# jimonld2000/AudioDenoiser

Measured on AMD Instinct MI355X. Metric: spectrogram frames/sec (forward), 513x256 fp32, higher is better.
Workload: dtype f32; 1 GPU; BASELINE configs[1]: batch=64 synthetic 513x256 fp32 spectrograms on one MI355X, full U-Net forward + per-clip perceptual loss; batch_per_gpu=64, global_batch=64, freq_bins=513, frames=256, parallelism=clips sharded over 1 rank(s), weights replicated, no data-path collective, lib_digest=616623384a0f

## Files before the change

### audiodenoiser_amd/csrc/adn_internal.h

```cpp
#pragma once
#include <hip/hip_runtime.h>
#include <atomic>
#include <cstddef>
#include <cstdint>
#include <type_traits>

namespace adn {

template <typename T> constexpr int ACT_BLOCK = 32 / (int)sizeof(T);
template <typename T>
__host__ __device__ __forceinline__ long act_off(int C, long HW, long pix, int c)
{
    constexpr int B = ACT_BLOCK<T>;
    (void)C;
    return ((long)(c / B) * HW + pix) * B + (c % B);
}

#ifdef __HIPCC__
typedef float f32x2 __attribute__((ext_vector_type(2)));
typedef float f32x4 __attribute__((ext_vector_type(4)));
typedef float f32x16 __attribute__((ext_vector_type(16)));
typedef _Float16 f16x2 __attribute__((ext_vector_type(2)));
typedef _Float16 f16x4 __attribute__((ext_vector_type(4)));
typedef _Float16 f16x8 __attribute__((ext_vector_type(8)));
// ... 207 lines not shown
}
inline int device_cus()
{
    static std::atomic<int> cus{0};
    int c = cus.load(std::memory_order_relaxed);
    if (c == 0) {
        int dev = 0;
        if (hipGetDevice(&dev) != hipSuccess || hipDeviceGetAttribute(&c, hipDeviceAttributeMultiprocessorCount, dev) != hipSuccess || c < 8)
            return 0;
        c &= ~7;
        cus.store(c, std::memory_order_relaxed);
    }
    return c;
}

hipError_t launch_conv_mfma(ConvKind kind, const ConvArgs &a, bool f16, hipStream_t st);
hipError_t launch_conv_reduce(ConvKind kind, const ConvArgs &a, bool f16, hipStream_t st);
hipError_t launch_convt_reduce(const float *partial, const float *bias, float *out, int ksplit, int N, int Ho, int Wo, int Cout,
                               hipStream_t st);
constexpr int WINO_BN = 32;
hipError_t launch_wino_conv(ConvKind kind, const ConvArgs &a, hipStream_t st);
long wino_tiles(ConvArgs &a);
bool wino4_applicable(ConvKind kind, const ConvArgs &a, bool force);
long wino4_workgroups(const ConvArgs &a);
hipError_t launch_wino4_conv(ConvKind kind, const ConvArgs &a, hipStream_t st);

struct Wino3sGeom {
    int tilesY, tilesX;
    long rows;
    size_t v_bytes, m_bytes;
    long gemm_grid;
};
enum SplitTile { SPLIT_BN128 = 0, SPLIT_BN256 = 1, SPLIT_BN256W8 = 2 };
inline int split_tile_bn(SplitTile t) { return t == SPLIT_BN128 ? 128 : 256; }
bool wino3s_applicable(ConvKind kind, const ConvArgs &a);
Wino3sGeom wino3s_geom(const ConvArgs &a);
hipError_t launch_wino3s_conv(ConvKind kind, const ConvArgs &a, float *V, float *M, SplitTile tile, hipStream_t st);
hipError_t launch_wino_gemm(const float *V, const void *U, float *M, long rows, int Cin, int Cout, SplitTile tile, hipStream_t st);

bool conv16_applicable(ConvKind kind, const ConvArgs &a);
hipError_t launch_conv16(ConvKind kind, const ConvArgs &a, bool resident, hipStream_t st);

bool convt16_applicable(const ConvArgs &a);
hipError_t launch_convt16(const ConvArgs &a, hipStream_t st);

hipError_t launch_conv_first(const float *x, const float *w9x64, const float *bias, void *out, bool f16,
                             int N, int H, int W, int Cin, hipStream_t st);
hipError_t launch_dot_finish(const float *planes, int nplanes, float bias, float *y, long npix, hipStream_t st);
hipError_t launch_conv_out(const void *in, bool f16, const float *w64, float bias, float *out, long npix, long HW,
                           long out_stride, hipStream_t st);
hipError_t launch_nhwc_to_nchw(const void *in, bool f16, float *out, int N, int H, int W, int C, hipStream_t st);

hipError_t launch_stft_mag(const float *audio, int n_clips, long L, int n_fft, int hop, int center, long n_frames,
// ... 204 lines not shown
```

### audiodenoiser_amd/csrc/conv_kernels.hip

```cpp
#include "adn_internal.h"

#include <cstdlib>

namespace adn {

namespace {

constexpr int TW = 16;
constexpr int CONVT_KG = 2, CONVT_WPE = 4;

template <typename T> struct Elem;
template <> struct Elem<float> { static constexpr int EPV = 4; };
template <> struct Elem<_Float16> { static constexpr int EPV = 8; };

template <int TH, int BN, int WM, int WN>
__device__ __forceinline__ void conv_epilogue_raw(const ConvArgs &p, f32x16 (&acc)[TH * TW / 32 / WM][BN / 32 / WN], int lane, int wave,
                                                  int ct, int n, int ty, int tx)
{
    constexpr int MB = TH * TW / 32 / WM, NB = BN / 32 / WN;
    const int wm = wave / WN, wn = wave % WN;
    const int hh = lane >> 5, l31 = lane & 31;
    float *ob = static_cast<float *>(p.out) + (size_t)n * p.H * p.W * p.Cout;
#pragma unroll
    for (int j = 0; j < NB; ++j) {
// ... 369 lines not shown
                    const T *b0 = stage + ((2 * ly) * TW + 2 * lx) * RS + part * EPP;
                    piece_t m = *reinterpret_cast<const piece_t *>(b0);
                    const piece_t m1 = *reinterpret_cast<const piece_t *>(b0 + RS);
                    const piece_t m2 = *reinterpret_cast<const piece_t *>(b0 + TW * RS);
                    const piece_t m3 = *reinterpret_cast<const piece_t *>(b0 + TW * RS + RS);
                    m = __builtin_elementwise_maximum(__builtin_elementwise_maximum(m, m1), __builtin_elementwise_maximum(m2, m3));
                    *reinterpret_cast<piece_t *>(poolp + (size_t)n * Hp * Wp * p.Cout +
                                                 act_off<T>(p.Cout, (long)Hp * Wp, (long)py * Wp + px, ct * BN + part * EPP)) = m;
                }
            }
        }
    }
    }
}

template <typename T, int TH, int BN, int WM, int WN, int TAPS, int KG, int SPLIT = 0>
struct DmaCfg {
    static constexpr int NT = 64 * WM * WN;
    static constexpr int HALO = (TAPS == 9) ? 1 : 0;
    static constexpr int PH = TH + 2 * HALO, PW = TW + 2 * HALO;
    static constexpr int KQ = 2 * KG;
    static constexpr int PSLOT = (KG == 1) ? KQ : KQ + 1;
    static constexpr int RSLOT = PW * PSLOT + ((KG == 1) ? 1 : 0);
    static constexpr int A_USED = PH * RSLOT;
    static constexpr int A_SLOTS = (A_USED + 63) / 64 * 64;
    static constexpr int B_SLOTS = SPLIT ? TAPS * 3 * 2 * BN : TAPS * KG * 2 * BN;
    static constexpr int SLOTS = A_SLOTS + B_SLOTS;
    static constexpr int NPIECE = (SLOTS + NT - 1) / NT;
    static constexpr int A_ROUNDS = (A_SLOTS + NT - 1) / NT;
    static constexpr size_t LDS_BYTES = (size_t)2 * SLOTS * 16;
    static_assert(B_SLOTS % 64 == 0, "weight slab must be a whole number of wave copies");
};

template <typename T, int TH, int BN, int WM, int WN, int TAPS, int KG, int EPI, int WPE, int SPLIT = 0, int KSPLIT = 0>
__global__ __launch_bounds__(64 * WM * WN, WPE) void conv_dma(const ConvArgs p)
{
    using C = DmaCfg<T, TH, BN, WM, WN, TAPS, KG, SPLIT>;
    static_assert(!KSPLIT || EPI == CONVT2X2 || (sizeof(T) == 2 && EPI == CONV3X3_RELU), "K split: transposed convolutions, fp16 3x3 layers");
    static_assert(!SPLIT || (sizeof(T) == 4 && KG == 2 && TAPS == 1), "SPLIT: fp32 storage, one 16-channel chunk (two fp32 k-groups), 1 tap");
    constexpr bool GEMM = EPI == WINO_GEMM;
    static_assert(!GEMM || (SPLIT && !KSPLIT && TW == 16), "Winograd GEMM stage: split-bf16 form");
    constexpr int NT = C::NT, EPV = Elem<T>::EPV, HALO = C::HALO, PW = C::PW;
    static_assert(2 * EPV == ACT_BLOCK<T>, "one k-group = one channel block of the activation layout");
    constexpr int PSLOT = C::PSLOT, RSLOT = C::RSLOT, A_SLOTS = C::A_SLOTS, SLOTS = C::SLOTS, NPIECE = C::NPIECE;
    constexpr int A_ROUNDS = C::A_ROUNDS;
    constexpr int B_DW = C::B_SLOTS * 4;
    constexpr int MB = TH * TW / 32 / WM, NB = BN / 32 / WN;
    static_assert(WM * WN == 4 || WM * WN == 8, "4 or 8 waves per workgroup");
    static_assert(MB >= 1 && NB >= 1, "tile too small");

    extern __shared__ __attribute__((aligned(16))) float smem[];

// ... 36 lines not shown
    unsigned cstr = (unsigned)((size_t)KG * src_hw(p.s0) * ACT_BLOCK<T> * sizeof(T));
    unsigned wsoff = 0;
    const int c0 = KSPLIT ? ksp * nloc : 0;
    bool in2 = false;
    if constexpr (KSPLIT) {
        wsoff = (unsigned)c0 * (unsigned)(B_DW * 4);
        if (c0 > p.nchunk0) {
            in2 = true;
            cstr = (unsigned)((size_t)KG * p.s1.H * p.s1.W * ACT_BLOCK<T> * sizeof(T));
            hptr = src_base(p.s1) + (size_t)(c0 - p.nchunk0) * cstr;
        } else {
            hptr += (size_t)c0 * cstr;
        }
    }
    const unsigned loff = lane * 16;
    unsigned hcur[A_ROUNDS];
    auto dma_piece = [&](int k, int buf, bool want_a, bool want_b) {
        const int sb = k * NT + wave * 64;
        if (sb >= SLOTS) return;
        float *dst = smem + (size_t)buf * SLOTS * 4 + sb * 4;
        if (k < A_ROUNDS && sb < A_SLOTS) {
            if (want_a) dma16_buf(dma_rsrc(hptr, cstr), hcur[k < A_ROUNDS ? k : 0], 0u, dst);
        } else if (want_b) {
            dma16_buf(wrs, loff, wsoff + (unsigned)(sb - A_SLOTS) * 16u, dst);
        }
    };
#pragma unroll
    for (int k = 0; k < NPIECE; ++k) dma_piece(k, 0, false, true);

    auto plan = [&](const ConvSrc &src) {
#pragma unroll
// ... 25 lines not shown
    float bias_r[NB];
#pragma unroll
    for (int j = 0; j < NB; ++j) bias_r[j] = GEMM ? 0.f : p.bias[ct * BN + (wn * NB + j) * 32 + l31];

    f32x16 acc[MB][NB];
#pragma unroll
    for (int i = 0; i < MB; ++i)
#pragma unroll
        for (int j = 0; j < NB; ++j)
#pragma unroll
            for (int r = 0; r < 16; ++r) acc[i][j][r] = 0.f;

    const int a_lane = ((wm * MB * 2 + ((lane >> 4) & 1)) * RSLOT + (lane & 15) * PSLOT) * 4 + hh * 4;
    const int b_lane = A_SLOTS * 4 + hh * BN * 4 + (wn * NB * 32 + l31) * 4;

    dma_chunk(c0, 0, false);
    asm volatile("s_waitcnt vmcnt(0)" ::: "memory");
    __syncthreads();
    for (int c = c0; c < c0 + nloc; ++c) {
        if (c + 1 < c0 + nloc) dma_chunk(c + 1, (c + 1 - c0) & 1);
        const float *img = smem + (size_t)((c - c0) & 1) * SLOTS * 4;
        if constexpr (SPLIT) {
            bf16x8 ah[MB], am[MB], al[MB];
#pragma unroll
            for (int i = 0; i < MB; ++i) {
                const float *ap = img + a_lane + (i * 2 * RSLOT) * 4 + hh * 4;
                split3_bf16(*reinterpret_cast<const f32x4 *>(ap), *reinterpret_cast<const f32x4 *>(ap + 4), ah[i], am[i], al[i]);
            }
#pragma unroll
            for (int j = 0; j < NB; ++j) {
// ... 31 lines not shown
#pragma unroll
                            for (int j = 0; j < NB; ++j)
                                acc[i][j] = __builtin_amdgcn_mfma_f32_32x32x2f32(a[i][kk], b[j][kk], acc[i][j], 0, 0, 0);
                } else {
#pragma unroll
                    for (int i = 0; i < MB; ++i)
#pragma unroll
                        for (int j = 0; j < NB; ++j)
                            acc[i][j] = __builtin_amdgcn_mfma_f32_32x32x16_f16(__builtin_bit_cast(f16x8, a[i]),
                                                                               __builtin_bit_cast(f16x8, b[j]), acc[i][j], 0, 0, 0);
                }
            }
        }
        asm volatile("s_waitcnt vmcnt(0)" ::: "memory");
        __syncthreads();
    }
    if constexpr (KSPLIT && EPI != CONVT2X2) {
        conv_epilogue_raw<TH, BN, WM, WN>(p, acc, lane, wave, ct, n + ksp * p.N, ty, tx);
    } else if constexpr (sizeof(T) == 2 || EPI == CONVT2X2 || GEMM) {
        constexpr size_t tile = (size_t)TH * TW * (BN + 16 / sizeof(T)) * sizeof(T);
        constexpr int HALVES = tile <= C::LDS_BYTES ? 1 : 2;
        static_assert(tile / HALVES <= C::LDS_BYTES, "staging tile (or half of it) must fit the two images");
        conv_epilogue_staged<T, TH, BN, WM, WN, EPI, HALVES>(p, acc, bias_r, smem, tid, lane, wave, ct, KSPLIT ? n + ksp * p.N : n, ty, tx);
    } else {
        conv_epilogue<T, TH, BN, WM, WN, EPI>(p, acc, bias_r, lane, wave, ct, n, ty, tx);
    }
}

constexpr int FIRST_ROWS = 8;

// ... 124 lines not shown
    }
}

template <typename T, int TH, int BN, int WM, int WN, int TAPS, int KG, int EPI>
hipError_t launch_cfg(const ConvArgs &a, hipStream_t st)
{
    constexpr int HALO = (TAPS == 9) ? 1 : 0;
    constexpr int PH = TH + 2 * HALO, PW = TW + 2 * HALO;
    constexpr size_t lds = (size_t)(PH * PW * (8 * KG + 4) + TAPS * KG * 2 * BN * 4) * sizeof(float);
    const long nwg = conv_workgroups(a);
    if (nwg <= 0 || nwg > 0x7fffffffL) return hipErrorInvalidValue;
    hipLaunchKernelGGL((conv_mfma<T, TH, BN, WM, WN, TAPS, KG, EPI>), dim3((unsigned)nwg), dim3(64 * WM * WN), lds, st, a);
    return hipGetLastError();
}

template <typename T, int TH, int BN, int WM, int WN, int TAPS, int KG, int EPI, int WPE, int SPLIT = 0, int KSPLIT = 0>
hipError_t launch_dma_cfg(const ConvArgs &a, hipStream_t st)
{
    using C = DmaCfg<T, TH, BN, WM, WN, TAPS, KG, SPLIT>;
    const long nwg = conv_workgroups(a);
    const int ks = KSPLIT ? a.ksplit : 1;
    if (nwg <= 0 || ks < 1 || nwg * ks > 0x7fffffffL || a.nchunk % ks) return hipErrorInvalidValue;
    ConvArgs a2 = a;
    a2.nwg_base = (int)nwg;
    a2.fdGc = a2.fdNcg = a2.fdTx = a2.fdTy = FastDiv{0u, 0u};
    const long maxd = a.nct > a.tilesX ? (a.nct > a.tilesY ? a.nct : a.tilesY) : (a.tilesX > a.tilesY ? a.tilesX : a.tilesY);
    if ((unsigned long long)nwg * (unsigned long long)maxd < 0x100000000ull) {
        a2.fdGc = make_fastdiv((unsigned)a.nct);
        a2.fdTx = make_fastdiv((unsigned)a.tilesX);
        a2.fdTy = make_fastdiv((unsigned)a.tilesY);
    }
    constexpr auto kern = conv_dma<T, TH, BN, WM, WN, TAPS, KG, EPI, WPE, SPLIT, KSPLIT>;
    if (C::LDS_BYTES > 64 * 1024) {
        const hipError_t e = lds_opt_in<kern>(C::LDS_BYTES);
        if (e != hipSuccess) return e;
    }
    hipLaunchKernelGGL(kern, dim3((unsigned)(nwg * ks)), dim3(C::NT), C::LDS_BYTES, st, a2);
    return hipGetLastError();
}

__global__ __launch_bounds__(256) void convt_reduce_kernel(const f32x4 *__restrict__ partial, const float *__restrict__ bias,
                                                           f32x4 *__restrict__ out, int ksplit, long n4, long hw, int cblocks)
{
    const long i = (long)blockIdx.x * 256 + threadIdx.x;
    if (i >= n4) return;
    const int c = (int)((i / (2 * hw)) % cblocks) * 8 + (int)(i & 1) * 4;
    f32x4 t[ADN_MAX_KSPLIT];
// ... 52 lines not shown
        for (int a = 0; a < 2; ++a)
#pragma unroll
            for (int b = 0; b < 2; ++b) {
                const int gy = 2 * by + a, gx = 2 * bx + b;
                if (gy >= H || gx >= W) continue;
                const f32x4 v = finish(gy, gx);
                mx.x = max_nan(mx.x, v.x); mx.y = max_nan(mx.y, v.y); mx.z = max_nan(mx.z, v.z); mx.w = max_nan(mx.w, v.w);
            }
        if (by < H / 2 && bx < W / 2)
            *reinterpret_cast<Tx4 *>(pool + (size_t)n * (H / 2) * (W / 2) * Cout +
                                     act_off<T>(Cout, (long)(H / 2) * (W / 2), (long)by * (W / 2) + bx, c4)) = as_t(mx);
    }
}

template <typename T>
hipError_t launch_conv_mfma_t(ConvKind kind, const ConvArgs &a, hipStream_t st)
{
    if constexpr (sizeof(T) == 2) {
        if (a.ksplit > 1) {
            if (kind != CONV3X3_RELU) return hipErrorInvalidValue;
            return launch_dma_cfg<T, 32, 64, 8, 1, 9, 1, CONV3X3_RELU, 4, 0, 1>(a, st);
        }
        if (kind == CONVT2X2) return launch_dma_cfg<T, 8, 128, 2, 2, 1, CONVT_KG, CONVT2X2, CONVT_WPE>(a, st);
        if (kind == CONV3X3_RELU_DOT) {
            if (a.nct != 1 || !a.dotw || !a.dot_out) return hipErrorInvalidValue;
            return launch_dma_cfg<T, 32, 64, 8, 1, 9, 1, CONV3X3_RELU_DOT, 4>(a, st);
        }
        if (kind == CONV3X3_RELU_POOL) return launch_dma_cfg<T, 32, 64, 8, 1, 9, 1, CONV3X3_RELU_POOL, 4>(a, st);
        return launch_dma_cfg<T, 32, 64, 8, 1, 9, 1, CONV3X3_RELU, 4>(a, st);
    } else {
        if (kind == CONV3X3_RELU_DOT) return hipErrorInvalidValue;
        if (kind == CONVT2X2) {
            if (a.split > 1 && a.ksplit > 1) return hipErrorInvalidValue;
            if (a.split && a.ksplit > 1) return launch_dma_cfg<T, 8, 128, 2, 2, 1, CONVT_KG, CONVT2X2, 3, 1, 1>(a, st);
            if (a.ksplit > 1) return hipErrorInvalidValue;
            if (a.split == 1 + SPLIT_BN256) return launch_dma_cfg<T, 8, 256, 2, 2, 1, CONVT_KG, CONVT2X2, 2, 1>(a, st);
            if (a.split == 1 + SPLIT_BN256W8) return launch_dma_cfg<T, 8, 256, 2, 4, 1, CONVT_KG, CONVT2X2, 2, 1>(a, st);
            if (a.split) return launch_dma_cfg<T, 8, 128, 2, 2, 1, CONVT_KG, CONVT2X2, 3, 1>(a, st);
            return launch_dma_cfg<T, 8, 128, 2, 2, 1, CONVT_KG, CONVT2X2, CONVT_WPE>(a, st);
        }
        if (a.Cout == 64) {
            if (kind == CONV3X3_RELU_POOL) return launch_cfg<T, 16, 64, 4, 1, 9, 1, CONV3X3_RELU_POOL>(a, st);
            return launch_cfg<T, 16, 64, 4, 1, 9, 1, CONV3X3_RELU>(a, st);
        }
        if (kind == CONV3X3_RELU_POOL) return launch_cfg<T, 8, 128, 2, 2, 9, 1, CONV3X3_RELU_POOL>(a, st);
        return launch_cfg<T, 8, 128, 2, 2, 9, 1, CONV3X3_RELU>(a, st);
    }
}
// ... 6 lines not shown
    if (kind == CONVT2X2) return ConvGeom{8, 128, CONVT_KG * cpg};
    if (f16) return ConvGeom{32, 64, cpg};
    if (Cout == 64) return ConvGeom{16, 64, cpg};
    return ConvGeom{8, 128, cpg};
}

long conv_mfma_tiles(ConvKind kind, bool f16, ConvArgs &a)
{
    const ConvGeom g = conv_geom(kind, a.Cout, f16);
    a.tilesY = (a.H + g.TH - 1) / g.TH;
    a.tilesX = (a.W + TW - 1) / TW;
    a.nct = (kind == CONVT2X2 ? 4 * a.Cout : a.Cout) / g.BN;
    return conv_workgroups(a);
}

hipError_t launch_conv_mfma(ConvKind kind, const ConvArgs &a, bool f16, hipStream_t st)
{
    return f16 ? launch_conv_mfma_t<_Float16>(kind, a, st) : launch_conv_mfma_t<float>(kind, a, st);
}

hipError_t launch_wino_gemm(const float *V, const void *U, float *M, long rows, int Cin, int Cout, SplitTile tile, hipStream_t st)
{
    const int BN = split_tile_bn(tile);
    if (!V || !U || !M || rows < 1 || rows >= (1L << 25) || Cin < 16 || (Cin & 15) || Cout < BN || Cout % BN) return hipErrorInvalidValue;
    ConvArgs a{};
    a.N = 36;
    a.W = TW;
    a.H = (int)((rows + TW - 1) / TW);
    a.rows = rows;
    a.s0 = ConvSrc{V, a.H, a.W, Cin, 0, 0};
    a.s1 = ConvSrc{V, 0, 0, 0, 0, 0};
    a.nchunk0 = a.nchunk = Cin / 16;
    a.wpk = U;
    a.out = M;
    a.Cout = Cout;
    a.ksplit = 1;
    a.split = 1;
    a.tilesY = (a.H + 7) / 8;
    a.tilesX = 1;
    a.nct = Cout / BN;
    if (tile == SPLIT_BN256) return launch_dma_cfg<float, 8, 256, 2, 2, 1, CONVT_KG, WINO_GEMM, 2, 1>(a, st);
    if (tile == SPLIT_BN256W8) return launch_dma_cfg<float, 8, 256, 2, 4, 1, CONVT_KG, WINO_GEMM, 2, 1>(a, st);
    return launch_dma_cfg<float, 8, 128, 2, 2, 1, CONVT_KG, WINO_GEMM, 3, 1>(a, st);
}

template <typename T>
static hipError_t launch_conv_reduce_t(bool pl, const ConvArgs &a, unsigned blocks, hipStream_t st)
{
    if (pl)
        hipLaunchKernelGGL((conv_reduce_kernel<T, true>), dim3(blocks), dim3(256), 0, st, a.partial, a.bias, static_cast<T *>(a.out),
                           static_cast<T *>(a.pool), a.ksplit, a.N, a.H, a.W, a.Cout);
    else
        hipLaunchKernelGGL((conv_reduce_kernel<T, false>), dim3(blocks), dim3(256), 0, st, a.partial, a.bias, static_cast<T *>(a.out),
                           static_cast<T *>(nullptr), a.ksplit, a.N, a.H, a.W, a.Cout);
    return hipGetLastError();
// ... 89 lines not shown
```

### audiodenoiser_amd/csrc/unet.hip

```cpp
#include "adn_host.h"

#include <algorithm>
#include <cmath>
#include <cstdlib>
#include <cstring>
#include <memory>
#include <vector>

using adn::aligned_to;
using adn::DeviceGuard;
using adn::fail;
using adn::fail_hip;

namespace {

constexpr float BN_EPS = 1e-5f;
constexpr int CH[5] = {64, 128, 256, 512, 1024};

enum LayerKind { CONV3, CONVT };
struct LayerDesc {
    LayerKind kind;
    int level;
    int C0, C1;
    int Cout;
// ... 49 lines not shown
    std::vector<hipEvent_t> events;
    int timing_max = 0, timing_count = 0;
    bool f16 = false;
    bool use_wino = true;
    bool use_wino4 = true, force_wino4 = false;
    bool allow_split = false;
    bool convt_split = true;
    int f16_conv = 1;
    int f16_convt = 1;
    bool f16_fuse_first = true;
    bool batch_invariant = false;
    long auto_grid = 192, auto_grid64 = 512;
    int wino_gemm = 1;
    long gemm_grid = 1536;
    int split_bn = -1;
    long convt_wide_grid = 2048;
};

namespace {

void bn_fold(const float *b, const float *gamma, const float *beta, const float *mean, const float *var, int C,
             std::vector<float> &scale, std::vector<float> &bias)
{
    scale.resize(C);
    bias.resize(C);
    for (int c = 0; c < C; ++c) {
        const float s = gamma[c] / std::sqrt(var[c] + BN_EPS);
        scale[c] = s;
        bias[c] = (b[c] - mean[c]) * s + beta[c];
    }
// ... 289 lines not shown
adn::ConvArgs convt_args(const adn_unet *h, const Plan &p, int i, const void *in, void *out)
{
    const LayerDesc &d = NET.v[i];
    const int H = p.H[d.level], W = p.W[d.level];
    adn::ConvArgs a = geom_args(d, h->f16, false, p.N, H, W);
    a.s0 = adn::ConvSrc{in, H, W, d.C0, 0, 0};
    a.s1 = adn::ConvSrc{in, 0, 0, 0, 0, 0};
    a.wpk = h->dev + h->lw[i].w_off;
    a.bias = h->dev + h->lw[i].b_off;
    a.out = out;
    a.split = h->convt_split ? 1 : 0;
    return a;
}


enum Conv3Kernel {
    DIRECT,
    CONV16,
    WINO2,
    WINO4,
    WINO3S
};
struct WinoScratch {
    const void *U = nullptr;
    adn::SplitTile tile = adn::SPLIT_BN128;
    float *V = nullptr, *M = nullptr;
    size_t v_bytes = 0, m_bytes = 0;
};
struct Conv3Choice {
    Conv3Kernel kernel;
    int ksplit;
    bool fuse_first;
    bool fuse_out;
};

Conv3Choice choose_conv3(const adn_unet *h, adn::ConvKind kind, const adn::ConvArgs &a, bool first = false, bool tail = false,
                         const WinoScratch &sc = WinoScratch())
{
    Conv3Choice c{DIRECT, 1, false, false};
    if (h->f16) {
// ... 52 lines not shown
                c.kernel = WINO4;
                c.ksplit = ks4;
            }
        }
    }
    return done();
}

hipError_t launch_conv3_kernels(const adn_unet *h, adn::ConvKind kind, const Conv3Choice &c, adn::ConvArgs a, float *partial, hipStream_t st,
                                const WinoScratch &sc)
{
    if (c.fuse_out) kind = adn::CONV3X3_RELU_DOT;
    switch (c.kernel) {
    case WINO3S:
        a.wpk = sc.U;
        return adn::launch_wino3s_conv(kind, a, sc.V, sc.M, sc.tile, st);
    case CONV16:
        a.wpk = a.wpk4;
        a.nchunk0 = a.s0.C / 32;
        a.nchunk = (a.s0.C + a.s1.C) / 32;
        if (c.fuse_first) a.nchunk0 = a.nchunk = 2;
        return adn::launch_conv16(kind, a, c.fuse_first || (a.s0.C + a.s1.C == 64 && a.Cout == 64), st);
    case DIRECT:
        if (c.ksplit > 1) {
            adn::ConvArgs sl = a;
            sl.ksplit = c.ksplit;
            sl.out = partial;
            sl.pool = nullptr;
            hipError_t e = adn::launch_conv_mfma(adn::CONV3X3_RELU, sl, true, st);
            if (e != hipSuccess) return e;
            a.ksplit = c.ksplit;
// ... 39 lines not shown
    int ksplit;
};

ConvTChoice choose_convt(const adn_unet *h, const LayerWeights &L, const adn::ConvArgs &a)
{
    ConvTChoice c{false, 1};
    if (h->f16) {
        c.t16 = L.w16_off && adn::convt16_applicable(a);
        return c;
    }
    if (h->convt_split && !h->batch_invariant)
        c.ksplit = adn::convt_ksplit(adn::conv_workgroups(a), a.nchunk, (size_t)a.N * (2 * a.H) * (2 * a.W) * a.Cout);
    return c;
}

hipError_t launch_convt_kernels(const adn_unet *h, const LayerWeights &L, const ConvTChoice &c, adn::ConvArgs a, float *partial, hipStream_t st)
{
    if (c.t16) {
        a.wpk = h->dev + L.w16_off;
        a.bias = h->dev + L.braw_off;
        return adn::launch_convt16(a, st);
    }
    if (c.ksplit > 1) {
        float *out = static_cast<float *>(a.out);
        a.ksplit = c.ksplit;
        a.out = partial;
        a.bias = h->dev + h->zero_off;
        hipError_t e = adn::launch_conv_mfma(adn::CONVT2X2, a, h->f16, st);
        if (e != hipSuccess) return e;
        return adn::launch_convt_reduce(partial, h->dev + L.braw_off, out, c.ksplit, a.N, 2 * a.H, 2 * a.W, a.Cout, st);
    }
    if (a.split && L.wt_off && (h->split_bn >= 0 || adn::conv_workgroups(a) >= h->convt_wide_grid)) {
        a.split = 1 + L.w3_tile;
        a.wpk = h->dev + L.wt_off;
        a.nct /= 2;
    }
    return adn::launch_conv_mfma(adn::CONVT2X2, a, h->f16, st);
}

int launch_convt(const adn_unet *h, int layer, const ConvTChoice &c, const adn::ConvArgs &a, float *partial, size_t part_bytes, hipStream_t st)
{
    if (int rc = check_part(layer, c.ksplit, (size_t)a.N * (2 * a.H) * (2 * a.W) * a.Cout, part_bytes)) return rc;
    return hip_status(launch_convt_kernels(h, h->lw[layer], c, a, partial, st), "launch_convt");
}


int forward_impl(adn_unet *h, const float *x, float *y, int N, int F, int T, void *workspace, size_t ws_bytes,
                 float *const *taps, hipStream_t st)
{
    if (!h || !x || !y) return fail(ADN_ERR_INVALID, "adn_unet_forward: null handle/x/y");
    Plan p;
    if (!make_plan(N, F, T, h->f16, p)) return fail(ADN_ERR_INVALID, "adn_unet_forward: need N>=1, F,T>=16 and F*T<2^27");
    if (!workspace || ws_bytes < p.total)
        return fail(ADN_ERR_WORKSPACE, "adn_unet_forward: workspace too small (see adn_unet_workspace_bytes)");
    if (!aligned_to(workspace, 16)) return fail(ADN_ERR_INVALID, "adn_unet_forward: workspace must be 16-byte aligned");
    if (!aligned_to(x, 4) || !aligned_to(y, 4)) return fail(ADN_ERR_INVALID, "adn_unet_forward: x and y must be 4-byte aligned");
    DeviceGuard guard(h->device);
    if (guard.err != hipSuccess) return fail_hip(guard.err, "hipSetDevice");
// ... 13 lines not shown
    auto export_tap = [&](int idx, const void *buf, int layer) -> hipError_t {
        if (!taps || !taps[idx]) return hipSuccess;
        const LayerDesc &d = NET.v[layer];
        return adn::launch_nhwc_to_nchw(buf, f16, taps[idx], N, p.H[d.level], p.W[d.level], d.Cout, st);
    };
    int i = 0;
    auto wino_scratch = [&](int li) {
        WinoScratch sc;
        const LayerDesc &d = NET.v[li];
        if (f16 || !h->lw[li].w3_off) return sc;
        const size_t full = (size_t)N * p.H[0] * p.W[0] * 64 * sizeof(float);
        const size_t front = (size_t)N * p.H[d.level] * p.W[d.level] * std::max(std::max(d.C0, d.C1), d.Cout) * sizeof(float);
        if (front >= full) return sc;
        sc.U = h->dev + h->lw[li].w3_off;
        sc.tile = h->lw[li].w3_tile;
        sc.V = reinterpret_cast<float *>(static_cast<char *>(tA) + front);
        sc.M = reinterpret_cast<float *>(static_cast<char *>(tB) + front);
        sc.v_bytes = sc.m_bytes = full - front;
        return sc;
    };

    const void *cur = tA;
    for (int l = 0; l < 4; ++l) {
        void *skip = ws + p.skip[l], *pool = ws + p.pool[l];
        if (l > 0) {
            const WinoScratch sc = wino_scratch(i);
            const adn::ConvArgs a = conv_args(h, p, i++, ws + p.pool[l - 1], nullptr, 0, 0, tA, nullptr);
            ADN_MARK();
            ADN_TRY(launch_conv3(h, i - 1, adn::CONV3X3_RELU, choose_conv3(h, adn::CONV3X3_RELU, a, false, false, sc), a, part, p.part_bytes, st, sc));
        }
// ... 97 lines not shown
    if (const char *algo = std::getenv("ADN_CONV_ALGO"))
        h.use_wino = std::strcmp(algo, "direct") != 0;
    if (h.f16) h.use_wino = false;
    if (const char *sk = std::getenv("ADN_WINO_SPLITK")) h.allow_split = std::atoi(sk) != 0;
    if (const char *cs = std::getenv("ADN_CONVT_SPLIT")) h.convt_split = std::atoi(cs) != 0;
    if (const char *bi = std::getenv("ADN_BATCH_INVARIANT")) h.batch_invariant = std::atoi(bi) != 0;
    if (const char *ff = std::getenv("ADN_F16_FIRST")) h.f16_fuse_first = std::atoi(ff) != 0;
    if (const char *fc = std::getenv("ADN_F16_CONV")) h.f16_conv = std::atoi(fc) == 32 ? 0 : 1;
    if (const char *ft = std::getenv("ADN_F16_CONVT")) h.f16_convt = std::strcmp(ft, "dma") == 0 ? 0 : 1;
    if (const char *ag = std::getenv("ADN_AUTO_GRID")) h.auto_grid = std::atol(ag);
    if (const char *ag = std::getenv("ADN_AUTO_GRID64")) h.auto_grid64 = std::atol(ag);
    if (h.f16) h.convt_split = false;
    if (const char *wg = std::getenv("ADN_WINO_GEMM")) h.wino_gemm = std::atoi(wg) == 2 ? 2 : std::atoi(wg) != 0;
    if (const char *sb = std::getenv("ADN_SPLIT_BN"))
        h.split_bn = !std::strcmp(sb, "128") ? adn::SPLIT_BN128 : !std::strcmp(sb, "256") ? adn::SPLIT_BN256 : !std::strcmp(sb, "256w8") ? adn::SPLIT_BN256W8 : -2;
    if (const char *wt = std::getenv("ADN_WINO_TILE")) {
        h.use_wino4 = std::atoi(wt) != 2;
        h.force_wino4 = std::atoi(wt) == 4;
    }
}

adn::SplitTile split_tile(const adn_unet &h, const LayerDesc &d)
{
    if ((d.kind == CONVT ? 4 * d.Cout : d.Cout) % 256) return adn::SPLIT_BN128;
    if (h.split_bn >= 0) return static_cast<adn::SplitTile>(h.split_bn);
    return d.kind == CONVT && d.Cout < 128 ? adn::SPLIT_BN128 : adn::SPLIT_BN256;
}

void pack_weights(adn_unet &h, const float *const *t, std::vector<float> &host)
{
// ... 130 lines not shown
int adn_unet_create_general(adn_unet **handle, int device, const float *const *t, int n_tensors, int dtype, int in_channels,
                            int num_classes)
{
    if (int rc = check_create_args(handle, device, t, n_tensors, dtype, in_channels, num_classes)) return rc;
    DeviceGuard guard(device);
    if (guard.err != hipSuccess) return fail_hip(guard.err, "hipSetDevice");
    if (int rc = check_device_arch(device)) return rc;

    std::unique_ptr<adn_unet, UnetDeleter> h(new adn_unet());
    h->device = device;
    h->in_ch = in_channels;
    h->n_classes = num_classes;
    h->f16 = dtype == ADN_DTYPE_F16;
    read_switches(*h);
    if (h->split_bn < -1) return fail(ADN_ERR_INVALID, "adn_unet_create: ADN_SPLIT_BN must be 128, 256 or 256w8");
    std::vector<float> host;
    pack_weights(*h, t, host);
    h->dev_floats = host.size();
    hipError_t e = hipMalloc(&h->dev, host.size() * sizeof(float));
    if (e != hipSuccess) return fail_hip(e, "hipMalloc(weights)");
    e = hipMemcpy(h->dev, host.data(), host.size() * sizeof(float), hipMemcpyHostToDevice);
    if (e != hipSuccess) return fail_hip(e, "hipMemcpy(weights)");
    *handle = h.release();
    return ADN_OK;
}

int adn_unet_set_timing(adn_unet *h, int max_forwards)
{
    if (!h || max_forwards < 0 || max_forwards > 4096) return fail(ADN_ERR_INVALID, "adn_unet_set_timing: bad argument");
    DeviceGuard guard(h->device);
// ... 51 lines not shown
```

### audiodenoiser_amd/csrc/wino3s_kernels.hip

```cpp
#include "adn_internal.h"

namespace adn {

namespace {

constexpr int NT = 256;

__global__ __launch_bounds__(NT) void wino3s_input_kernel(const ConvArgs p, float *__restrict__ V, int tilesY, int tilesX, long rows)
{
    const long id = (long)blockIdx.x * NT + threadIdx.x;
    const long row = id >> 1;
    const int half = (int)(id & 1), cb = blockIdx.y;
    if (row >= rows) return;
    const int tx = (int)(row % tilesX);
    const long r2 = row / tilesX;
    const int ty = (int)(r2 % tilesY), n = (int)(r2 / tilesY);
    const bool second = cb >= p.s0.C / 8;
    const ConvSrc &s = second ? p.s1 : p.s0;
    const int cbl = second ? cb - p.s0.C / 8 : cb;
    const float *src = static_cast<const float *>(s.ptr) + ((size_t)n * (s.C / 8) + cbl) * ((size_t)s.H * s.W * 8) + half * 4;
    const int y0 = 4 * ty - 1 - s.offY, x0 = 4 * tx - 1 - s.offX;
    f32x4 d[6][6];
#pragma unroll
    for (int a = 0; a < 6; ++a)
// ... 80 lines not shown
    return a.N >= 1 && a.H >= 1 && a.W >= 1 && wino3s_geom(a).rows < (1L << 25);
}

Wino3sGeom wino3s_geom(const ConvArgs &a)
{
    Wino3sGeom g{};
    g.tilesY = (a.H + 3) / 4;
    g.tilesX = (a.W + 3) / 4;
    g.rows = (long)a.N * g.tilesY * g.tilesX;
    g.v_bytes = (size_t)36 * g.rows * (a.s0.C + a.s1.C) * sizeof(float);
    g.m_bytes = (size_t)36 * g.rows * a.Cout * sizeof(float);
    g.gemm_grid = 36 * ((g.rows + 127) / 128) * (a.Cout / 128);
    return g;
}

hipError_t launch_wino3s_conv(ConvKind kind, const ConvArgs &a, float *V, float *M, SplitTile tile, hipStream_t st)
{
    if (!wino3s_applicable(kind, a) || !V || !M || !a.wpk || !a.bias || !a.out) return hipErrorInvalidValue;
    const Wino3sGeom g = wino3s_geom(a);
    const long bx = (2 * g.rows + NT - 1) / NT;
    const int Cin = a.s0.C + a.s1.C;
    hipLaunchKernelGGL(wino3s_input_kernel, dim3((unsigned)bx, (unsigned)(Cin / 8)), dim3(NT), 0, st, a, V, g.tilesY, g.tilesX, g.rows);
    hipError_t e = hipGetLastError();
    if (e != hipSuccess) return e;
    e = launch_wino_gemm(V, a.wpk, M, g.rows, Cin, a.Cout, tile, st);
    if (e != hipSuccess) return e;
    if (kind == CONV3X3_RELU_POOL)
        hipLaunchKernelGGL(wino3s_output_kernel<true>, dim3((unsigned)bx, (unsigned)(a.Cout / 8)), dim3(NT), 0, st, a, M, g.tilesY,
                           g.tilesX, g.rows);
    else
        hipLaunchKernelGGL(wino3s_output_kernel<false>, dim3((unsigned)bx, (unsigned)(a.Cout / 8)), dim3(NT), 0, st, a, M, g.tilesY,
                           g.tilesX, g.rows);
    return hipGetLastError();
}

}
```

Measured before the change: 525,300 frames/s.

## Feed split-bf16 A operand from registers via direct buffer loads

```diff
diff --git a/audiodenoiser_amd/csrc/adn_internal.h b/audiodenoiser_amd/csrc/adn_internal.h
--- a/audiodenoiser_amd/csrc/adn_internal.h
+++ b/audiodenoiser_amd/csrc/adn_internal.h
@@ -245,7 +245,8 @@
     return c;
 }
 
-hipError_t launch_conv_mfma(ConvKind kind, const ConvArgs &a, bool f16, hipStream_t st);
+enum SplitA { SPLIT_A_LDS = 0, SPLIT_A_REG = 1 };
+hipError_t launch_conv_mfma(ConvKind kind, const ConvArgs &a, bool f16, hipStream_t st, SplitA afeed = SPLIT_A_LDS);
 hipError_t launch_conv_reduce(ConvKind kind, const ConvArgs &a, bool f16, hipStream_t st);
 hipError_t launch_convt_reduce(const float *partial, const float *bias, float *out, int ksplit, int N, int Ho, int Wo, int Cout,
                                hipStream_t st);
@@ -266,8 +267,8 @@
 inline int split_tile_bn(SplitTile t) { return t == SPLIT_BN128 ? 128 : 256; }
 bool wino3s_applicable(ConvKind kind, const ConvArgs &a);
 Wino3sGeom wino3s_geom(const ConvArgs &a);
-hipError_t launch_wino3s_conv(ConvKind kind, const ConvArgs &a, float *V, float *M, SplitTile tile, hipStream_t st);
-hipError_t launch_wino_gemm(const float *V, const void *U, float *M, long rows, int Cin, int Cout, SplitTile tile, hipStream_t st);
+hipError_t launch_wino3s_conv(ConvKind kind, const ConvArgs &a, float *V, float *M, SplitTile tile, SplitA afeed, hipStream_t st);
+hipError_t launch_wino_gemm(const float *V, const void *U, float *M, long rows, int Cin, int Cout, SplitTile tile, SplitA afeed, hipStream_t st);
 
 bool conv16_applicable(ConvKind kind, const ConvArgs &a);
 hipError_t launch_conv16(ConvKind kind, const ConvArgs &a, bool resident, hipStream_t st);
diff --git a/audiodenoiser_amd/csrc/conv_kernels.hip b/audiodenoiser_amd/csrc/conv_kernels.hip
--- a/audiodenoiser_amd/csrc/conv_kernels.hip
+++ b/audiodenoiser_amd/csrc/conv_kernels.hip
@@ -407,7 +407,7 @@
     }
 }
 
-template <typename T, int TH, int BN, int WM, int WN, int TAPS, int KG, int SPLIT = 0>
+template <typename T, int TH, int BN, int WM, int WN, int TAPS, int KG, int SPLIT = 0, int AREG = 0>
 struct DmaCfg {
     static constexpr int NT = 64 * WM * WN;
     static constexpr int HALO = (TAPS == 9) ? 1 : 0;
@@ -416,19 +416,21 @@
     static constexpr int PSLOT = (KG == 1) ? KQ : KQ + 1;
     static constexpr int RSLOT = PW * PSLOT + ((KG == 1) ? 1 : 0);
     static constexpr int A_USED = PH * RSLOT;
-    static constexpr int A_SLOTS = (A_USED + 63) / 64 * 64;
+    static constexpr int A_SLOTS = AREG ? 0 : (A_USED + 63) / 64 * 64;
     static constexpr int B_SLOTS = SPLIT ? TAPS * 3 * 2 * BN : TAPS * KG * 2 * BN;
     static constexpr int SLOTS = A_SLOTS + B_SLOTS;
     static constexpr int NPIECE = (SLOTS + NT - 1) / NT;
     static constexpr int A_ROUNDS = (A_SLOTS + NT - 1) / NT;
-    static constexpr size_t LDS_BYTES = (size_t)2 * SLOTS * 16;
+    static constexpr size_t STAGE_HALF = (size_t)TH * TW * (BN + 16 / sizeof(T)) * sizeof(T) / 2;
+    static constexpr size_t LDS_BYTES = AREG && STAGE_HALF > (size_t)2 * SLOTS * 16 ? STAGE_HALF : (size_t)2 * SLOTS * 16;
     static_assert(B_SLOTS % 64 == 0, "weight slab must be a whole number of wave copies");
 };
 
-template <typename T, int TH, int BN, int WM, int WN, int TAPS, int KG, int EPI, int WPE, int SPLIT = 0, int KSPLIT = 0>
+template <typename T, int TH, int BN, int WM, int WN, int TAPS, int KG, int EPI, int WPE, int SPLIT = 0, int KSPLIT = 0, int AREG = 0>
 __global__ __launch_bounds__(64 * WM * WN, WPE) void conv_dma(const ConvArgs p)
 {
-    using C = DmaCfg<T, TH, BN, WM, WN, TAPS, KG, SPLIT>;
+    using C = DmaCfg<T, TH, BN, WM, WN, TAPS, KG, SPLIT, AREG>;
+    static_assert(!AREG || (AREG == 1 && SPLIT && WM * WN == 4 && WM == 2), "AREG: split-bf16 form on the 4-wave tiles");
     static_assert(!KSPLIT || EPI == CONVT2X2 || (sizeof(T) == 2 && EPI == CONV3X3_RELU), "K split: transposed convolutions, fp16 3x3 layers");
     static_assert(!SPLIT || (sizeof(T) == 4 && KG == 2 && TAPS == 1), "SPLIT: fp32 storage, one 16-channel chunk (two fp32 k-groups), 1 tap");
     constexpr bool GEMM = EPI == WINO_GEMM;
@@ -495,7 +497,7 @@
         }
     }
     const unsigned loff = lane * 16;
-    unsigned hcur[A_ROUNDS];
+    unsigned hcur[A_ROUNDS ? A_ROUNDS : 1];
     auto dma_piece = [&](int k, int buf, bool want_a, bool want_b) {
         const int sb = k * NT + wave * 64;
         if (sb >= SLOTS) return;
@@ -551,6 +553,86 @@
     const int a_lane = ((wm * MB * 2 + ((lane >> 4) & 1)) * RSLOT + (lane & 15) * PSLOT) * 4 + hh * 4;
     const int b_lane = A_SLOTS * 4 + hh * BN * 4 + (wn * NB * 32 + l31) * 4;
 
+    if constexpr (AREG) {
+        const int cend = c0 + nloc;
+        unsigned aoff[MB];
+        auto aplan = [&](const ConvSrc &src) {
+#pragma unroll
+            for (int i = 0; i < MB; ++i) {
+                const int y0 = gy0 + (wm * MB + i) * 2 + (l31 >> 4) - src.offY, x0 = gx0 + (l31 & 15) - src.offX;
+                aoff[i] = (y0 >= 0 && y0 < src.H && x0 >= 0 && x0 < src.W && (!GEMM || (long)y0 * src.W + x0 < p.rows))
+                              ? (unsigned)act_off<T>(src.C, (long)src_hw(src), y0 * src.W + x0, hh * 2 * EPV) * (unsigned)sizeof(T) : ADN_DMA_OOB;
+            }
+        };
+        f32x4 raw[MB][2];
+        auto a_load = [&](int c) {
+            if (c == p.nchunk0 && c < cend) {
+                hptr = src_base(p.s1);
+                cstr = (unsigned)((size_t)KG * p.s1.H * p.s1.W * ACT_BLOCK<T> * sizeof(T));
+                aplan(p.s1);
+            }
+            const unsigned kill = c < cend ? 0u : ADN_DMA_OOB;
+            const __amdgpu_buffer_rsrc_t ars = dma_rsrc(hptr, cstr);
+#pragma unroll
+            for (int i = 0; i < MB; ++i) {
+                raw[i][0] = __builtin_bit_cast(f32x4, __builtin_amdgcn_raw_buffer_load_b128(ars, aoff[i] | kill, 0, 0));
+                raw[i][1] = __builtin_bit_cast(f32x4, __builtin_amdgcn_raw_buffer_load_b128(ars, aoff[i] | 16u | kill, 0, 0));
+            }
+            hptr += cstr;
+        };
+        static_assert(SLOTS % NT == 0, "every wave sends NPIECE copies per chunk: the counted waits below rely on it");
+        auto b_copy = [&](int buf, unsigned kill) {
+#pragma unroll
+            for (int k = 0; k < NPIECE; ++k) {
+                const int sb = k * NT + wave * 64;
+                dma16_buf(wrs, loff | kill, wsoff + (unsigned)sb * 16u, smem + (size_t)buf * SLOTS * 4 + sb * 4);
+            }
+            wsoff += B_DW * 4;
+        };
+        wsoff += B_DW * 4;
+        if (in2) aplan(p.s1);
+        else aplan(p.s0);
+        bf16x8 ah[MB], am[MB], al[MB];
+        a_load(c0);
+#pragma unroll
+        for (int i = 0; i < MB; ++i) split3_bf16(raw[i][0], raw[i][1], ah[i], am[i], al[i]);
+        a_load(c0 + 1);
+        asm volatile("s_waitcnt vmcnt(%0)" ::"n"(2 * MB) : "memory");
+        __syncthreads();
+        for (int c = c0; c < cend; ++c) {
+            b_copy((c + 1 - c0) & 1, c + 1 < cend ? 0u : ADN_DMA_OOB);
+            const float *img = smem + (size_t)((c - c0) & 1) * SLOTS * 4;
+            bf16x8 nh[MB], nm[MB], nl[MB];
+#pragma unroll
+            for (int j = 0; j < NB; ++j) {
+                const bf16x8 bh = __builtin_bit_cast(bf16x8, *reinterpret_cast<const f32x4 *>(img + b_lane + j * 128));
+                const bf16x8 bm = __builtin_bit_cast(bf16x8, *reinterpret_cast<const f32x4 *>(img + b_lane + j * 128 + 2 * BN * 4));
+                const bf16x8 bl = __builtin_bit_cast(bf16x8, *reinterpret_cast<const f32x4 *>(img + b_lane + j * 128 + 4 * BN * 4));
+#pragma unroll
+                for (int i = 0; i < MB; ++i) {
+                    acc[i][j] = __builtin_amdgcn_mfma_f32_32x32x16_bf16(al[i], bh, acc[i][j], 0, 0, 0);
+                    acc[i][j] = __builtin_amdgcn_mfma_f32_32x32x16_bf16(ah[i], bl, acc[i][j], 0, 0, 0);
+                    acc[i][j] = __builtin_amdgcn_mfma_f32_32x32x16_bf16(am[i], bm, acc[i][j], 0, 0, 0);
+                    acc[i][j] = __builtin_amdgcn_mfma_f32_32x32x16_bf16(am[i], bh, acc[i][j], 0, 0, 0);
+                    acc[i][j] = __builtin_amdgcn_mfma_f32_32x32x16_bf16(ah[i], bm, acc[i][j], 0, 0, 0);
+                    acc[i][j] = __builtin_amdgcn_mfma_f32_32x32x16_bf16(ah[i], bh, acc[i][j], 0, 0, 0);
+                }
+                if (j == 0) {
+#pragma unroll
+                    for (int i = 0; i < MB; ++i) split3_bf16(raw[i][0], raw[i][1], nh[i], nm[i], nl[i]);
+                    a_load(c + 2);
+                }
+            }
+            asm volatile("s_waitcnt vmcnt(%0)" ::"n"(2 * MB) : "memory");
+            __syncthreads();
+#pragma unroll
+            for (int i = 0; i < MB; ++i) {
+                ah[i] = nh[i];
+                am[i] = nm[i];
+                al[i] = nl[i];
+            }
+        }
+    } else {
     dma_chunk(c0, 0, false);
     asm volatile("s_waitcnt vmcnt(0)" ::: "memory");
     __syncthreads();
@@ -612,6 +694,7 @@
         }
         asm volatile("s_waitcnt vmcnt(0)" ::: "memory");
         __syncthreads();
+    }
     }
     if constexpr (KSPLIT && EPI != CONVT2X2) {
         conv_epilogue_raw<TH, BN, WM, WN>(p, acc, lane, wave, ct, n + ksp * p.N, ty, tx);
@@ -766,10 +849,10 @@
     return hipGetLastError();
 }
 
-template <typename T, int TH, int BN, int WM, int WN, int TAPS, int KG, int EPI, int WPE, int SPLIT = 0, int KSPLIT = 0>
+template <typename T, int TH, int BN, int WM, int WN, int TAPS, int KG, int EPI, int WPE, int SPLIT = 0, int KSPLIT = 0, int AREG = 0>
 hipError_t launch_dma_cfg(const ConvArgs &a, hipStream_t st)
 {
-    using C = DmaCfg<T, TH, BN, WM, WN, TAPS, KG, SPLIT>;
+    using C = DmaCfg<T, TH, BN, WM, WN, TAPS, KG, SPLIT, AREG>;
     const long nwg = conv_workgroups(a);
     const int ks = KSPLIT ? a.ksplit : 1;
     if (nwg <= 0 || ks < 1 || nwg * ks > 0x7fffffffL || a.nchunk % ks) return hipErrorInvalidValue;
@@ -782,7 +865,7 @@
         a2.fdTx = make_fastdiv((unsigned)a.tilesX);
         a2.fdTy = make_fastdiv((unsigned)a.tilesY);
     }
-    constexpr auto kern = conv_dma<T, TH, BN, WM, WN, TAPS, KG, EPI, WPE, SPLIT, KSPLIT>;
+    constexpr auto kern = conv_dma<T, TH, BN, WM, WN, TAPS, KG, EPI, WPE, SPLIT, KSPLIT, AREG>;
     if (C::LDS_BYTES > 64 * 1024) {
         const hipError_t e = lds_opt_in<kern>(C::LDS_BYTES);
         if (e != hipSuccess) return e;
@@ -865,9 +948,10 @@
 }
 
 template <typename T>
-hipError_t launch_conv_mfma_t(ConvKind kind, const ConvArgs &a, hipStream_t st)
+hipError_t launch_conv_mfma_t(ConvKind kind, const ConvArgs &a, SplitA afeed, hipStream_t st)
 {
     if constexpr (sizeof(T) == 2) {
+        if (afeed != SPLIT_A_LDS) return hipErrorInvalidValue;
         if (a.ksplit > 1) {
             if (kind != CONV3X3_RELU) return hipErrorInvalidValue;
             return launch_dma_cfg<T, 32, 64, 8, 1, 9, 1, CONV3X3_RELU, 4, 0, 1>(a, st);
@@ -881,8 +965,15 @@
         return launch_dma_cfg<T, 32, 64, 8, 1, 9, 1, CONV3X3_RELU, 4>(a, st);
     } else {
         if (kind == CONV3X3_RELU_DOT) return hipErrorInvalidValue;
+        if (afeed != SPLIT_A_LDS && kind != CONVT2X2) return hipErrorInvalidValue;
         if (kind == CONVT2X2) {
             if (a.split > 1 && a.ksplit > 1) return hipErrorInvalidValue;
+            if (afeed == SPLIT_A_REG) {
+                if (!a.split || a.split == 1 + SPLIT_BN256W8) return hipErrorInvalidValue;
+                if (a.ksplit > 1) return launch_dma_cfg<T, 8, 128, 2, 2, 1, CONVT_KG, CONVT2X2, 3, 1, 1, 1>(a, st);
+                if (a.split == 1 + SPLIT_BN256) return launch_dma_cfg<T, 8, 256, 2, 2, 1, CONVT_KG, CONVT2X2, 2, 1, 0, 1>(a, st);
+                return launch_dma_cfg<T, 8, 128, 2, 2, 1, CONVT_KG, CONVT2X2, 3, 1, 0, 1>(a, st);
+            }
             if (a.split && a.ksplit > 1) return launch_dma_cfg<T, 8, 128, 2, 2, 1, CONVT_KG, CONVT2X2, 3, 1, 1>(a, st);
             if (a.ksplit > 1) return hipErrorInvalidValue;
             if (a.split == 1 + SPLIT_BN256) return launch_dma_cfg<T, 8, 256, 2, 2, 1, CONVT_KG, CONVT2X2, 2, 1>(a, st);
@@ -919,13 +1010,14 @@
     return conv_workgroups(a);
 }
 
-hipError_t launch_conv_mfma(ConvKind kind, const ConvArgs &a, bool f16, hipStream_t st)
-{
-    return f16 ? launch_conv_mfma_t<_Float16>(kind, a, st) : launch_conv_mfma_t<float>(kind, a, st);
-}
-
-hipError_t launch_wino_gemm(const float *V, const void *U, float *M, long rows, int Cin, int Cout, SplitTile tile, hipStream_t st)
-{
+hipError_t launch_conv_mfma(ConvKind kind, const ConvArgs &a, bool f16, hipStream_t st, SplitA afeed)
+{
+    return f16 ? launch_conv_mfma_t<_Float16>(kind, a, afeed, st) : launch_conv_mfma_t<float>(kind, a, afeed, st);
+}
+
+hipError_t launch_wino_gemm(const float *V, const void *U, float *M, long rows, int Cin, int Cout, SplitTile tile, SplitA afeed, hipStream_t st)
+{
+    if (afeed == SPLIT_A_REG && tile == SPLIT_BN256W8) return hipErrorInvalidValue;
     const int BN = split_tile_bn(tile);
     if (!V || !U || !M || rows < 1 || rows >= (1L << 25) || Cin < 16 || (Cin & 15) || Cout < BN || Cout % BN) return hipErrorInvalidValue;
     ConvArgs a{};
@@ -944,6 +1036,10 @@
     a.tilesY = (a.H + 7) / 8;
     a.tilesX = 1;
     a.nct = Cout / BN;
+    if (afeed == SPLIT_A_REG) {
+        if (tile == SPLIT_BN256) return launch_dma_cfg<float, 8, 256, 2, 2, 1, CONVT_KG, WINO_GEMM, 2, 1, 0, 1>(a, st);
+        return launch_dma_cfg<float, 8, 128, 2, 2, 1, CONVT_KG, WINO_GEMM, 3, 1, 0, 1>(a, st);
+    }
     if (tile == SPLIT_BN256) return launch_dma_cfg<float, 8, 256, 2, 2, 1, CONVT_KG, WINO_GEMM, 2, 1>(a, st);
     if (tile == SPLIT_BN256W8) return launch_dma_cfg<float, 8, 256, 2, 4, 1, CONVT_KG, WINO_GEMM, 2, 1>(a, st);
     return launch_dma_cfg<float, 8, 128, 2, 2, 1, CONVT_KG, WINO_GEMM, 3, 1>(a, st);
diff --git a/audiodenoiser_amd/csrc/unet.hip b/audiodenoiser_amd/csrc/unet.hip
--- a/audiodenoiser_amd/csrc/unet.hip
+++ b/audiodenoiser_amd/csrc/unet.hip
@@ -87,6 +87,7 @@
     int wino_gemm = 1;
     long gemm_grid = 1536;
     int split_bn = -1;
+    int split_a = -1;
     long convt_wide_grid = 2048;
 };
 
@@ -406,6 +407,14 @@
 }
 
 
+adn::SplitA split_afeed(const adn_unet &h, const LayerDesc &d, adn::SplitTile tile)
+{
+    if (tile == adn::SPLIT_BN256W8) return adn::SPLIT_A_LDS;
+    if (h.split_a >= 0) return static_cast<adn::SplitA>(h.split_a);
+    if (tile != adn::SPLIT_BN256) return adn::SPLIT_A_LDS;
+    return d.kind == CONVT || d.C1 == 0 ? adn::SPLIT_A_REG : adn::SPLIT_A_LDS;
+}
+
 enum Conv3Kernel {
     DIRECT,
     CONV16,
@@ -416,6 +425,7 @@
 struct WinoScratch {
     const void *U = nullptr;
     adn::SplitTile tile = adn::SPLIT_BN128;
+    adn::SplitA afeed = adn::SPLIT_A_LDS;
     float *V = nullptr, *M = nullptr;
     size_t v_bytes = 0, m_bytes = 0;
 };
@@ -498,7 +508,7 @@
     switch (c.kernel) {
     case WINO3S:
         a.wpk = sc.U;
-        return adn::launch_wino3s_conv(kind, a, sc.V, sc.M, sc.tile, st);
+        return adn::launch_wino3s_conv(kind, a, sc.V, sc.M, sc.tile, sc.afeed, st);
     case CONV16:
         a.wpk = a.wpk4;
         a.nchunk0 = a.s0.C / 32;
@@ -568,7 +578,8 @@
     return c;
 }
 
-hipError_t launch_convt_kernels(const adn_unet *h, const LayerWeights &L, const ConvTChoice &c, adn::ConvArgs a, float *partial, hipStream_t st)
+hipError_t launch_convt_kernels(const adn_unet *h, const LayerDesc &d, const LayerWeights &L, const ConvTChoice &c, adn::ConvArgs a, float *partial,
+                                hipStream_t st)
 {
     if (c.t16) {
         a.wpk = h->dev + L.w16_off;
@@ -580,7 +591,7 @@
         a.ksplit = c.ksplit;
         a.out = partial;
         a.bias = h->dev + h->zero_off;
-        hipError_t e = adn::launch_conv_mfma(adn::CONVT2X2, a, h->f16, st);
+        hipError_t e = adn::launch_conv_mfma(adn::CONVT2X2, a, h->f16, st, a.split ? split_afeed(*h, d, adn::SPLIT_BN128) : adn::SPLIT_A_LDS);
         if (e != hipSuccess) return e;
         return adn::launch_convt_reduce(partial, h->dev + L.braw_off, out, c.ksplit, a.N, 2 * a.H, 2 * a.W, a.Cout, st);
     }
@@ -589,13 +600,13 @@
         a.wpk = h->dev + L.wt_off;
         a.nct /= 2;
     }
-    return adn::launch_conv_mfma(adn::CONVT2X2, a, h->f16, st);
+    return adn::launch_conv_mfma(adn::CONVT2X2, a, h->f16, st, a.split ? split_afeed(*h, d, static_cast<adn::SplitTile>(a.split - 1)) : adn::SPLIT_A_LDS);
 }
 
 int launch_convt(const adn_unet *h, int layer, const ConvTChoice &c, const adn::ConvArgs &a, float *partial, size_t part_bytes, hipStream_t st)
 {
     if (int rc = check_part(layer, c.ksplit, (size_t)a.N * (2 * a.H) * (2 * a.W) * a.Cout, part_bytes)) return rc;
-    return hip_status(launch_convt_kernels(h, h->lw[layer], c, a, partial, st), "launch_convt");
+    return hip_status(launch_convt_kernels(h, NET.v[layer], h->lw[layer], c, a, partial, st), "launch_convt");
 }
 
 
@@ -639,6 +650,7 @@
         if (front >= full) return sc;
         sc.U = h->dev + h->lw[li].w3_off;
         sc.tile = h->lw[li].w3_tile;
+        sc.afeed = split_afeed(*h, d, sc.tile);
         sc.V = reinterpret_cast<float *>(static_cast<char *>(tA) + front);
         sc.M = reinterpret_cast<float *>(static_cast<char *>(tB) + front);
         sc.v_bytes = sc.m_bytes = full - front;
@@ -766,6 +778,8 @@
     if (const char *wg = std::getenv("ADN_WINO_GEMM")) h.wino_gemm = std::atoi(wg) == 2 ? 2 : std::atoi(wg) != 0;
     if (const char *sb = std::getenv("ADN_SPLIT_BN"))
         h.split_bn = !std::strcmp(sb, "128") ? adn::SPLIT_BN128 : !std::strcmp(sb, "256") ? adn::SPLIT_BN256 : !std::strcmp(sb, "256w8") ? adn::SPLIT_BN256W8 : -2;
+    if (const char *sa = std::getenv("ADN_SPLIT_A"))
+        h.split_a = !std::strcmp(sa, "lds") ? adn::SPLIT_A_LDS : !std::strcmp(sa, "reg") ? adn::SPLIT_A_REG : -2;
     if (const char *wt = std::getenv("ADN_WINO_TILE")) {
         h.use_wino4 = std::atoi(wt) != 2;
         h.force_wino4 = std::atoi(wt) == 4;
@@ -926,6 +940,7 @@
     h->f16 = dtype == ADN_DTYPE_F16;
     read_switches(*h);
     if (h->split_bn < -1) return fail(ADN_ERR_INVALID, "adn_unet_create: ADN_SPLIT_BN must be 128, 256 or 256w8");
+    if (h->split_a < -1) return fail(ADN_ERR_INVALID, "adn_unet_create: ADN_SPLIT_A must be lds or reg");
     std::vector<float> host;
     pack_weights(*h, t, host);
     h->dev_floats = host.size();
diff --git a/audiodenoiser_amd/csrc/wino3s_kernels.hip b/audiodenoiser_amd/csrc/wino3s_kernels.hip
--- a/audiodenoiser_amd/csrc/wino3s_kernels.hip
+++ b/audiodenoiser_amd/csrc/wino3s_kernels.hip
@@ -118,7 +118,7 @@
     return g;
 }
 
-hipError_t launch_wino3s_conv(ConvKind kind, const ConvArgs &a, float *V, float *M, SplitTile tile, hipStream_t st)
+hipError_t launch_wino3s_conv(ConvKind kind, const ConvArgs &a, float *V, float *M, SplitTile tile, SplitA afeed, hipStream_t st)
 {
     if (!wino3s_applicable(kind, a) || !V || !M || !a.wpk || !a.bias || !a.out) return hipErrorInvalidValue;
     const Wino3sGeom g = wino3s_geom(a);
@@ -127,7 +127,7 @@
     hipLaunchKernelGGL(wino3s_input_kernel, dim3((unsigned)bx, (unsigned)(Cin / 8)), dim3(NT), 0, st, a, V, g.tilesY, g.tilesX, g.rows);
     hipError_t e = hipGetLastError();
     if (e != hipSuccess) return e;
-    e = launch_wino_gemm(V, a.wpk, M, g.rows, Cin, a.Cout, tile, st);
+    e = launch_wino_gemm(V, a.wpk, M, g.rows, Cin, a.Cout, tile, afeed, st);
     if (e != hipSuccess) return e;
     if (kind == CONV3X3_RELU_POOL)
         hipLaunchKernelGGL(wino3s_output_kernel<true>, dim3((unsigned)bx, (unsigned)(a.Cout / 8)), dim3(NT), 0, st, a, M, g.tilesY,
```

Result: no change. 528,000 frames/s (median of 6 runs) (+0.5%).
